# giech/usrp_nfc

Measured on AMD Instinct MI355X. Metric: IQ Msamples/s -> decoded bits (2 Msps stream), higher is better.
Workload: dtype f32 envelope / f64 window sums / u8 symbols; 1 GPU; configs[1]: Miller-only decode, synthetic IQ @2 Msps; input_kind=fc32 IQ, 8 B/sample (envelope computed in the kernel), samples_per_gpu=100000000, parallelism=time-chunk x1, edges_per_gpu=6627699, symbols_reader=3971547, symbols_tag=0, packets=101186, boundary_redos=0, exchange=none, stepping=sync, in_flight=1

## Files before the change

usrp_nfc_amd/csrc/host_context.h:

```cpp
#pragma once


namespace {

std::string g_create_error;

}

enum : int {
    TOT_RUNS = 0,
    TOT_EDGES = 8,
    TOT_DECMAP = 16,
    TOT_SPEC = 40,
    TOT_PKT0 = 72,
    TOT_PKT1 = 80,
    TOT_LAST2 = 88,
    TOT_NSYM = 96,
    TOT_CERT = 104,
    TOT_FRAME = 128,
    TOT_BYTES = 160
};

static_assert(sizeof(CertSummary) <= TOT_FRAME - TOT_CERT, "the verdict summary fits its slot of the totals");
struct DevState {
    Carry carry;
    EdgeCarry ecarry;
    DecCarry dcarry;
    uint8_t totals[TOT_BYTES];
    uint32_t seq[4];
};

constexpr size_t AHEAD_LDS_MAX = 96 * 1024;
constexpr int LEAN_STEPS_AHEAD = 4;
constexpr int NRING = 4;
constexpr int NSUB = 3;

namespace {
struct Switches {
    std::optional<std::string> debug_clk;
    std::optional<int> no_small, debug_bad_launch, debug_redo_submitted, debug, trace, trace_alloc, no_submit_ahead, wg, wg_rounds, wg_bulk, wg_rerun, wg_rowbal, wg_nr, wg_per_cu, wg_per_cu_ahead, wg_ex, lean, lean_rounds,
        lean_waves, edge_prefix, dec_spec, dec_runin, spin_wait, chunk_adapt, chunk_mult;
    std::optional<double> lean_gfac, lean_gmin, eps;
    std::optional<unsigned long> own_prefix_max;
    std::optional<std::pair<int, int>> wg_lone;
    std::optional<std::array<double, 3>> rowbal_f;
    std::optional<bool> ring_global;
};
inline Switches read_switches() {
    Switches s;
#ifdef NFC_TEST_HOOKS
    const struct { const char *name; std::optional<int> Switches::*at; } ints[] = {
        {"NFC_NO_SMALL", &Switches::no_small}, {"NFC_DEBUG_BAD_LAUNCH", &Switches::debug_bad_launch}, {"NFC_DEBUG_REDO_SUBMITTED", &Switches::debug_redo_submitted},
        {"NFC_DEBUG", &Switches::debug}, {"NFC_TRACE", &Switches::trace}, {"NFC_TRACE_ALLOC", &Switches::trace_alloc}, {"NFC_NO_SUBMIT_AHEAD", &Switches::no_submit_ahead},
        {"NFC_WG", &Switches::wg}, {"NFC_WG_ROUNDS", &Switches::wg_rounds}, {"NFC_WG_BULK", &Switches::wg_bulk},
        {"NFC_WG_RERUN", &Switches::wg_rerun}, {"NFC_WG_NR", &Switches::wg_nr}, {"NFC_WG_PER_CU", &Switches::wg_per_cu},
        {"NFC_WG_PER_CU_AHEAD", &Switches::wg_per_cu_ahead}, {"NFC_WG_EX", &Switches::wg_ex}, {"NFC_LEAN", &Switches::lean}, {"NFC_LEAN_ROUNDS", &Switches::lean_rounds},
        {"NFC_LEAN_WAVES", &Switches::lean_waves}, {"NFC_EDGE_PREFIX", &Switches::edge_prefix}, {"NFC_DEC_SPEC", &Switches::dec_spec}, {"NFC_DEC_RUNIN", &Switches::dec_runin},
        {"NFC_SPIN_WAIT", &Switches::spin_wait}, {"NFC_CHUNK_ADAPT", &Switches::chunk_adapt}, {"NFC_CHUNK_MULT", &Switches::chunk_mult}};
    const struct { const char *name; std::optional<double> Switches::*at; } reals[] = {
        {"NFC_LEAN_GFAC", &Switches::lean_gfac}, {"NFC_LEAN_GMIN", &Switches::lean_gmin}, {"NFC_EPS", &Switches::eps}};
    for (const auto &v : ints)
        if (const char *e = getenv(v.name)) s.*v.at = atoi(e);
    for (const auto &v : reals)
        if (const char *e = getenv(v.name)) s.*v.at = atof(e);
    if (const char *e = getenv("NFC_DEBUG_CLK")) s.debug_clk = e;
    if (const char *e = getenv("NFC_OWN_PREFIX_MAX")) s.own_prefix_max = strtoul(e, nullptr, 10);
    if (const char *e = getenv("NFC_WG_LONE")) {
        int a = 4, b = 64;
        if (sscanf(e, "%d,%d", &a, &b) >= 1) s.wg_lone = std::make_pair(a, b);
    }
    if (const char *e = getenv("NFC_WG_ROWBAL")) {
        std::array<double, 3> f{0.0, 1.0, 1.0};
        if (sscanf(e, "%lf,%lf,%lf", &f[0], &f[1], &f[2]) >= 2 && f[0] > 0.5 && f[0] < 1.5 && f[1] > 0.5 && f[1] < 1.5 && f[2] > 0.5 && f[2] < 1.5)
            s.rowbal_f = f;
        else s.wg_rowbal = atoi(e);
    }
    if (const char *e = getenv("NFC_RING")) {
        if (strcmp(e, "global") == 0) s.ring_global = true;
        else if (strcmp(e, "lds") == 0) s.ring_global = false;
    }
#endif
// ... 92 lines not shown
    uint32_t slot_next = 0;
    bool low_valid = false;
    size_t lean_lds_per_cu = 0;
    size_t ahead_lds_per_cu = 0;
    uint32_t stamp_b = 0;
    bool in_wait = false;
    uint32_t dbg_fast_waits = 0;
    uint32_t stats_redo_submitted = 0;
    Carry h_carry;
    EdgeCarry h_ecarry;
    DecCarry h_dcarry;
    uint64_t nseen = 0;

    DevBuf d_certinfo;
    DevBuf d_in, d_neg, d_pos, d_ringout[2], d_touched[2], d_info[2], d_ringin, d_meta, d_ver, d_cflags, d_list;
    DevBuf d_ecode, d_epos, d_eidx;
    bool edges_from_host = false;
    std::vector<nfc_edge> h_pushed;
    DevBuf d_states, d_sym[2], d_bits[2], d_pending[2][2], d_close_end[2],
        d_close_idx[2];
    DevBuf d_partials, d_partials2, d_aggs, d_faggs;
    DevBuf d_edge_rec;
    int edge_prefix = -1;
    DevBuf d_spec;
    DevBuf d_stage_bits[2], d_stage_cb[2], d_stage_ci[2], d_stage_q[2], d_stage_own;
    DevBuf d_pack;
    DevBuf d_gvtop;
    DevBuf d_seqout;
    uint32_t cap_edges = 0, cap_sym[2] = {0, 0};
    uint32_t alloc_edges = 0, alloc_sym[2] = {0, 0};
    uint64_t alloc_mark = 0;
    uint64_t cap_edges_floor = 0, cap_sym_floor[2] = {0, 0};
    double edge_rate = 0.125;
    double sym_rate[2] = {1.0, 2.0};
    int pend_cur = 0;
    std::vector<uint8_t> h_ver;
    std::vector<uint32_t> h_list;

    const void *last_in = nullptr;
    uint32_t last_n = 0, last_skip = 0;
    uint64_t last_g0 = 0;
    uint32_t n_edges = 0;
    uint32_t n_sym[2] = {0, 0}, n_close[2] = {0, 0}, n_bits[2] = {0, 0};
    bool have_outputs = false;
    nfc_stats stats;
    std::vector<nfc_packet> pk[2];
// ... 80 lines not shown
#define HIPCHK(c, call)                                                                              \
    do {                                                                                             \
        hipError_t e__ = (call);                                                                     \
        if (e__ != hipSuccess)                                                                       \
            return fail((c), NFC_ERR_DEVICE, "%s failed: %s (%s:%d)", #call, hipGetErrorString(e__), __FILE__, __LINE__); \
    } while (0)

int batch_ok(nfc_ctx *c, bool with_mirror) {
    LaunchError &le = launch_error();
    if (le.err != hipSuccess) {
        const LaunchError e = le;
        le = LaunchError{};
        return fail(c, NFC_ERR_DEVICE, "kernel launch failed: %s (%s:%d)", hipGetErrorString(e.err), e.file, e.line);
    }
    if (with_mirror && c->hs->seq[0] != c->batch_seq)
        return fail(c, NFC_ERR_DEVICE, "state mirror is stale (batch %u, mirror %u): a kernel of this batch did not run", c->batch_seq, c->hs->seq[0]);
    return NFC_OK;
}
#define BATCHCHK(c, with_mirror)                                   \
    do {                                                           \
        if (int rc__ = batch_ok((c), (with_mirror))) return rc__;  \
    } while (0)

void launch_fill_kind(nfc_ctx *c, const void *in, uint32_t n, int nchunks, int ring_idx = -1) {
    float *ring = c->d_ring[ring_idx < 0 ? c->ring_cur : ring_idx].as<float>();
    Carry *cr = dC(c);
    EdgeCarryInit eci{(int32_t *)dE(c), c->L % c->mx};
    uint8_t *ver = c->d_ver.as<uint8_t>();
    CertSummary *sum = (CertSummary *)(dT(c) + TOT_CERT);
    StateInit init;
    memset(&init, 0, sizeof init);
    int fresh = 0;
    if (c->state_dirty) {
        static_assert(offsetof(DevState, totals) <= sizeof init.words && offsetof(DevState, totals) % 4 == 0, "state head fits");
        DevState h;
        h.carry = c->dirty_carry;
        h.ecarry = c->dirty_ecarry;
        h.dcarry = c->dirty_dcarry;
        init.apply = 1;
        init.n_words = (int32_t)(offsetof(DevState, totals) / 4);
        memcpy(init.words, &h, offsetof(DevState, totals));
        init.dst = (uint32_t *)c->d_state.p;
        init.fill_ring = c->dirty_fill_ring ? 1 : 0;
        init.fill = c->dirty_fill;
        init.ring_len = c->Lpad;
        c->state_dirty = c->dirty_fill_ring = false;
        fresh = h.carry.stable == 0 && h.carry.filled == 0 && n >= (uint32_t)c->L && (void *)cr == c->d_state.p;
// ... 21 lines not shown
```

usrp_nfc_amd/csrc/host_threshold.h:

```cpp
#pragma once

namespace {

static bool sums_exact(const Carry &hc, int emin, int emax, uint32_t vtop) {
    int low = emin - 23;
    if (hc.ss_emin != 255) low = std::min(low, hc.ss_emin);
    float vtf;
    memcpy(&vtf, &vtop, 4);
    int high = 255 + 64;
    if (std::isfinite(vtf) && vtf >= 0.f) high = vtf > 0.f ? std::ilogb((double)vtf) + 127 : 0;
    high = std::max(high, hc.ss_emax);
    return (emax < 255) && (high - low <= 52);
}

static inline void eps_adapt(nfc_ctx *c, const CertSummary &s) {
    if (!c->dbg_trace) return;
    float w;
    memcpy(&w, &s.worst, 4);
    fprintf(stderr, "[nfc] eps %.5f: the speculation used %.5f of the window sum at most, %u chunks failed their certification\n", (double)c->eps, (double)w, s.n_fail);
}

static inline void cpu_relax() {
#if defined(__x86_64__) || defined(__i386__)
    __builtin_ia32_pause();
// ... 236 lines not shown
    P.h_gflags = h_gflags;
    P.h_gmin = h_gmin;
    P.h_gmax = h_gmax;
    return NFC_OK;
}

static void enqueue_pass0(nfc_ctx *c, const ThrPlan &P, ThrArgs &A, const Event *own_events = nullptr) {
    A.list = nullptr;
    A.nlist = 0;
    A.mode = 0;
    A.cert = P.d_cert;
    A.sum = (CertSummary *)(dT(c) + TOT_CERT);
    A.ksteps = P.form == ThrForm::Workgroup ? c->wg_rounds : c->lean_rounds;
    A.gfac = c->lean_gfac;
    A.gfloor = c->lean_gmin;
    A.blk = 1 << c->nfold;
    launch_threshold(c, P, ThrLaunch::Pass0, A, P.nch, own_events);
}
static void enqueue_certify(nfc_ctx *c, const ThrPlan &P, const ThrArgs &A, CertInfo *info, float *ring_out, CertSummary *sum) {
    NFC_LAUNCH(k_certify, dim3(cert_grid(A.nlist)), dim3(256), 0, c->st, A, P.d_cert, info, ring_out, dC(c), sum);
}

static int threshold_span(nfc_ctx *c, const void *d_in_all, uint32_t n_all, uint32_t skip_all, uint32_t base, const EdgeCarry &ec,
                          const std::function<int()> *ahead, bool *clean, bool *need_seq_out, bool *recut_out = nullptr) {
    bool ran_ahead = false;
    *clean = false;
    const int L = c->L;
    const uint32_t n = n_all - base;
    const uint32_t skip = skip_all > base ? skip_all - base : 0u;
    const void *d_in = (const char *)d_in_all + (size_t)base * c->in_bytes_per_sample;
    const uint64_t nseen = c->nseen + base;
    uint32_t passes = 0;
    ThrArgs A;
    ThrPlan P;
    if (int rc = thr_prepare(c, d_in, n, n_all, skip, base, nseen, ec, c->ring_cur, c->d_neg, c->d_pos, false, A, P)) return rc;
    const uint32_t nch = P.nch;
    const bool wg = P.form == ThrForm::Workgroup;
    uint8_t *d_cert = P.d_cert;
    const uint8_t *h_cert = P.h_cert, *h_gflags = P.h_gflags, *h_gmin = P.h_gmin, *h_gmax = P.h_gmax;

    launch_fill_kind(c, d_in, n, (int)nch);

    const bool force_seq = (c->P.flags & NFC_FLAG_FORCE_SEQUENTIAL) != 0 || L < STEP;
    bool need_seq = force_seq;
    if (!force_seq) {
        const bool lean = wg || P.form == ThrForm::Lean;
        const bool dbg_clk = lean && c->dbg_clk;
        if (dbg_clk) {
            HIPCHK(c, c->d_certinfo.ensure((size_t)nch * 32 * 5));
            A.dbg_clk = c->d_certinfo.as<unsigned long long>();
        }
        enqueue_pass0(c, P, A);
        if (dbg_clk) {
            std::vector<unsigned long long> h((size_t)nch * 4);
            HIPCHK(c, hipStreamSynchronize(c->st));
            HIPCHK(c, hipMemcpy(h.data(), c->d_certinfo.p, (size_t)nch * 32, hipMemcpyDeviceToHost));
            unsigned long long t0 = ~0ull, t1 = 0;
            double pro = 0, loop = 0, epi = 0, maxtot = 0, maxstart = 0;
            for (uint32_t k = 0; k < nch; k++) {
                t0 = std::min(t0, h[4 * k]);
                t1 = std::max(t1, h[4 * k + 3]);
            }
            for (uint32_t k = 0; k < nch; k++) {
                pro += (double)(h[4 * k + 1] - h[4 * k]);
                loop += (double)(h[4 * k + 2] - h[4 * k + 1]);
                epi += (double)(h[4 * k + 3] - h[4 * k + 2]);
                maxtot = std::max(maxtot, (double)(h[4 * k + 3] - h[4 * k]));
                maxstart = std::max(maxstart, (double)(h[4 * k] - t0));
            }
#ifdef NFC_WG_PROF
            if (wg) {
                std::vector<unsigned long long> pf((size_t)nch * 16);
                HIPCHK(c, hipMemcpy(pf.data(), (char *)c->d_certinfo.p + (size_t)nch * 32, (size_t)nch * 128, hipMemcpyDeviceToHost));
                double tk = 0, b1 = 0, b2 = 0, rr = 0;
                for (size_t k = 0; k < (size_t)nch * 4; k++) {
// ... 62 lines not shown
                    HIPCHK(c, mirror_async(c));
                } else {
                    stamped_last = c->timing < 2;
                }
                if (rc) return rc;
                ran_ahead = true;
            } else {
                launch_certify();
                flags_with_verdict = first_round && c->fine_left > 0;
                if (!first_round || flags_with_verdict) {
                    HIPCHK(c, hipMemcpyAsync(c->h_cflags.p, c->d_cflags.p, (size_t)4 * nch, hipMemcpyDeviceToHost, c->st));
                    HIPCHK(c, hipMemcpyAsync(P.h_gvtop, c->d_gvtop.p, (size_t)nch * 4, hipMemcpyDeviceToHost, c->st));
                }
                HIPCHK(c, mirror_async(c));
                if (first_round && ahead) {
                    const int rc = (*ahead)();
                    if (rc) return rc;
                    ran_ahead = true;
                }
            }
            if (stamped_last) HIPCHK(c, wait_for_stamp(c));
            else HIPCHK(c, hipStreamSynchronize(c->st));
            BATCHCHK(c, true);
            std::vector<uint32_t> failing;
            if (first_round) {
                memcpy(&summary, c->hs->totals + TOT_CERT, sizeof summary);
                if (base == 0) eps_adapt(c, summary);
                if (summary.n_fail == 0 && !dbg) {
                    have_summary = true;
                    break;
                }
                if (recut_out && c->fine_adapt && wg && c->fine_left == 0 && !c->P.chunk_samples && c->fine_mult > 1 &&
                    (uint64_t)summary.n_fail * 64u > (uint64_t)nch) {
                    *recut_out = true;
                    A.ver_zero = 0;
                    return NFC_OK;
                }
                if (!flags_with_verdict) HIPCHK(c, hipMemcpy(c->h_cflags.p, c->d_cflags.p, (size_t)4 * nch, hipMemcpyDeviceToHost));
            }
            if (first_round && lean && !h_cert[0]) failing.push_back(0);
            for (uint32_t k : c->h_list)
                if (!h_cert[k]) failing.push_back(k);
            if (c->dbg_trace) {
                fprintf(stderr, "[nfc] round %d: n_fail %u, %zu failing of %u pending (cert[0] %d):", rounds, summary.n_fail, failing.size(), np, (int)h_cert[0]);
                for (size_t i = 0; i < failing.size() && i < 12; i++) fprintf(stderr, " %u(%x)", failing[i], (unsigned)h_gflags[failing[i]]);
                int why[8] = {0};
// ... 173 lines not shown
    if (ec_out) {
        int32_t o[3];
        HIPCHK(c, hipStreamSynchronize(c->st));
        HIPCHK(c, hipMemcpy(o, c->d_seqout.p, sizeof o, hipMemcpyDeviceToHost));
        ec_out->state = o[0];
        ec_out->last_bit = o[1];
        ec_out->dur = o[2];
    }
    return NFC_OK;
}

int run_threshold(nfc_ctx *c, const void *d_in, uint32_t n, uint32_t skip, const std::function<int()> *ahead, bool *clean) {
    *clean = false;
    c->stats.threshold_passes = 0;
    c->stats.chunks_rerun = 0;
    c->stats.chunks_rerun_in_place = 0;
    c->stats.used_sequential = 0;
    const uint32_t span = (uint32_t)std::min<uint64_t>(((uint64_t)8 * c->L + STEP - 1) / STEP * STEP, 1u << 30);
    EdgeCarry ec = c->h_ecarry;
    uint32_t base = 0;
    for (int round = 0;; round++) {
        bool need_seq = false, span_clean = false;
        const bool optimistic = base == 0 && !(c->fine_adapt && c->fine_left > 0);
        bool recut = false;
        int rc = threshold_span(c, d_in, n, skip, base, ec, optimistic ? ahead : nullptr, &span_clean, &need_seq, &recut);
        if (rc) return rc;
        if (recut) {
            c->fine_left = 8;
            c->cert_pending = false;
            HIPCHK(c, hipMemsetAsync((char *)dC(c) + offsetof(Carry, fin_valid), 0, sizeof(int32_t), c->st));
            span_clean = false;
            rc = threshold_span(c, d_in, n, skip, base, ec, nullptr, &span_clean, &need_seq, nullptr);
            if (rc) return rc;
        }
        if (!need_seq) {
            *clean = span_clean && base == 0;
            if (c->fine_adapt) {
                if ((uint64_t)c->stats.chunks_rerun * 64u > (uint64_t)c->stats.n_chunks) c->fine_left = 8;
                else if (c->fine_left > 0) c->fine_left--;
            }
            return NFC_OK;
        }
        const bool forced = (c->P.flags & NFC_FLAG_FORCE_SEQUENTIAL) != 0 || c->L < STEP;
        const uint32_t left = n - base;
        if (forced || round >= 6 || left <= 4 * span) return sequential_span(c, d_in, skip, base, left, ec, nullptr);
        const int rs = sequential_span(c, d_in, skip, base, span, ec, &ec);
        if (rs) return rs;
        base += span;
    }
// ... 5 lines not shown
```

usrp_nfc_amd/csrc/nfc_amd.hip:

```cpp
#include <hip/hip_runtime.h>
#include <hip/hip_ext.h>

#include <algorithm>
#include <atomic>
#include <chrono>
#include <cmath>
#include <cstdarg>
#include <cstdio>
#include <cstdlib>
#include <cstring>
#include <string>
#include <thread>
#include <array>
#include <functional>
#include <memory>
#include <optional>
#include <vector>

#include "../../include/nfc_amd.h"
#include "launch_check.h"
#include "decode.hip.h"
#include "decoder_tables.h"
#include "edges.hip.h"
#include "scan.hip.h"
// ... 62 lines not shown
    c->use_small = sw.no_small ? 0 : 1;
    c->dbg_bad_launch = sw.debug_bad_launch.has_value();
    c->dbg_redo_submitted = sw.debug_redo_submitted.has_value();
    c->dbg_any = sw.debug.has_value();
    c->dbg_trace = sw.trace.has_value();
    devbuf_trace() = sw.trace_alloc.has_value();
    if (sw.debug_clk) {
        c->dbg_clk = true;
        c->dbg_clk_path = *sw.debug_clk;
    }
    c->dbg_no_submit_ahead = sw.no_submit_ahead.has_value();
    if (sw.wg) c->wg = *sw.wg != 0;
    if (sw.wg_rounds) c->wg_rounds = std::max(1, *sw.wg_rounds);
    if (sw.wg_bulk) c->wg_bulk = *sw.wg_bulk != 0;
    if (sw.wg_rerun) c->wg_rerun_lone = *sw.wg_rerun != 0;
    if (sw.wg_lone) c->wg_lone_max = std::max(0, sw.wg_lone->first), c->wg_lone_div = std::max(1, sw.wg_lone->second);
    if (sw.lean) c->lean = *sw.lean != 0;
    c->lean_rounds = 0;
    if (sw.lean_rounds) c->lean_rounds = std::max(1, *sw.lean_rounds);
    if (sw.lean_gfac) c->lean_gfac = (float)*sw.lean_gfac;
    if (sw.lean_gmin) c->lean_gmin = (float)*sw.lean_gmin;
    if (sw.own_prefix_max) c->own_prefix_max = (uint32_t)*sw.own_prefix_max;
    if (sw.edge_prefix) c->edge_prefix = *sw.edge_prefix != 0;
    if (sw.dec_spec) c->dec_spec = *sw.dec_spec != 0;
    if (sw.spin_wait) c->spin_wait = *sw.spin_wait != 0;
    if (sw.rowbal_f) memcpy(c->rowbal_f[0], sw.rowbal_f->data(), sizeof c->rowbal_f[0]), c->rowbal_set = true;
    if (sw.wg_rowbal) c->wg_rowbal = *sw.wg_rowbal != 0;
    if (sw.dec_runin) c->dec_runin = *sw.dec_runin >= 2048 ? 8 : (*sw.dec_runin >= 1024 ? 4 : 2);
    C = (C + STEP - 1) / STEP * STEP;
    c->C_min = C;
    c->lds_per_slot = (p->input_kind == NFC_IN_ENV_F32) ? 5 : 4;
    c->wpb = std::max(1, std::min(4, (int)(65536 / ((size_t)c->Lpad * c->lds_per_slot))));
    c->gring_ok = (size_t)c->Lpad * c->lds_per_slot > 12 * 1024 && c->L >= 2 * STEP;
    if (sw.ring_global) {
        if (*sw.ring_global && c->L >= 2 * STEP) c->gring_ok = c->gring_force = 1;
        else if (!*sw.ring_global) c->gring_ok = 0;
    }
    c->hi_plus = p->hi_val + 0.1;
    const double eps = std::ldexp(1.0, -48);
    auto band = [&](double v, double &a, double &b) {
        a = v - std::fabs(v) * eps;
        b = v + std::fabs(v) * eps;
    };
    band(p->lo_val, c->lo_a, c->lo_b);
    band(p->hi_val, c->hi_a, c->hi_b);
    auto sane = [](double v) { return v == 0 || (std::fabs(v) > 1e-100 && std::fabs(v) < 1e100); };
// ... 154 lines not shown
    }
    c->T.mil_map = c->d_mil_map.as<uint4>();
    c->T.man_map = c->d_man_map.as<uint2>();
    c->T.mil_step = c->d_mil_out.as<uint16_t>();
    c->T.man_step = c->d_man_out.as<uint16_t>();
    c->T.nd = c->mx + 1;
    c->T.reader = p->enable_reader ? 1 : 0;
    c->T.tag = p->enable_tag ? 1 : 0;
    for (int k = 0; k < 3; k++) c->dec_lds[k] = dec_table_bytes((DecLdsUser)k, c->T);
    CRT(c->d_state.ensure(sizeof(DevState)));
    CRT(c->hs_pin.ensure(sizeof(DevState)));
    c->hs = c->hs_pin.as<DevState>();
    memset(c->hs, 0, sizeof(DevState));
    CRT(hipHostGetDevicePointer(&c->hs_dev, c->hs, 0));
    for (int b = 0; b < NRING; b++) {
        CRT(c->d_ring[b].ensure((size_t)c->Lpad * 4));
        CRT(hipMemset(c->d_ring[b].p, 0, (size_t)c->Lpad * 4));
    }
    for (int b = 0; b < 2; b++) {
        CRT(c->d_pending[b][0].ensure(1024));
        CRT(c->d_pending[b][1].ensure(1024));
    }
    push_state(c, 1);
    CRT(hipStreamSynchronize(c->st));
    return NFC_OK;
}
#undef CRT
}

extern "C" {

int nfc_abi_version(void) { return NFC_AMD_ABI_VERSION; }

int nfc_plan_row_cut(uint32_t n, uint32_t C, uint32_t rs, uint32_t cus, uint32_t rows, const double *factors, uint32_t max_len, uint32_t out[10]) {
    if (!out || !rs || !C || !cus || (rows >= 2 && !factors)) return NFC_ERR_ARG;
    const RowCut t = (rows >= 2 && rows <= 4) ? plan_row_cut(n, C, rs, cus, rows, factors, max_len) : equal_cut(n, C, cus);
    for (int r = 0; r < 4; r++) {
        out[r] = t.row_len[r];
        out[4 + r] = t.row_start[r];
    }
    out[8] = t.row_div;
    out[9] = t.nch;
    return t.by_row ? 1 : 0;
}

int nfc_device_count(void) {
// ... 947 lines not shown
#ifdef NFC_GEN_PROF
extern "C" int nfc_debug_gen_prof(unsigned long long *out, int reset) {
    const size_t bytes = sizeof(unsigned long long) * 8192 * 8;
    if (hipMemcpyFromSymbol(out, HIP_SYMBOL(nfc::g_gen_prof), bytes) != hipSuccess) return -1;
    {
        unsigned long long ri[2] = {0, 0};
        if (hipMemcpyFromSymbol(ri, HIP_SYMBOL(nfc::g_row_iters), sizeof ri) == hipSuccess)
            fprintf(stderr, "[nfc] row_exact: %llu rows, %.2f iterations each\n", ri[0], ri[0] ? (double)ri[1] / (double)ri[0] : 0.0);
        void *q = nullptr;
        if (reset && hipGetSymbolAddress(&q, HIP_SYMBOL(nfc::g_row_iters)) == hipSuccess) (void)hipMemset(q, 0, sizeof ri);
    }
    if (reset) {
        void *p = nullptr;
        if (hipGetSymbolAddress(&p, HIP_SYMBOL(nfc::g_gen_prof)) != hipSuccess || hipMemset(p, 0, bytes) != hipSuccess) return -1;
    }
    return 0;
}
#endif
#ifdef NFC_TEST_HOOKS
extern "C" float nfc_debug_frames_ms(const nfc_ctx *c) { return c && c->frames_ready ? c->fr_ms : -1.f; }
extern "C" void nfc_debug_live_resources(uint64_t out[4]) {
    for (int k = 0; k < 4; k++) out[k] = nfc::live::count(k).load();
}
extern "C" int nfc_debug_dec_lds(const nfc_ctx *c, int which, uint32_t *dyn_bytes, int *wgs_per_cu) {
    if (!c || which < 0 || which > 2 || !dyn_bytes || !wgs_per_cu) return NFC_ERR_ARG;
    const bool lds = 4 * c->T.nd <= nfc::DEC_LDS_ROWS;
    const void *k = which == 0   ? (const void *)nfc::dec_spec_kernel(lds, c->T)
                    : which == 1 ? (lds ? (const void *)nfc::k_dec_reduce<true> : (const void *)nfc::k_dec_reduce<false>)
                                 : (lds ? (const void *)nfc::k_dec_apply<true> : (const void *)nfc::k_dec_apply<false>);
    *dyn_bytes = (uint32_t)c->dec_lds[which];
    if (hipSetDevice(c->P.device) != hipSuccess) return NFC_ERR_DEVICE;
    return hipOccupancyMaxActiveBlocksPerMultiprocessor(wgs_per_cu, k, nfc::SCAN_BLOCK, c->dec_lds[which]) == hipSuccess ? NFC_OK : NFC_ERR_DEVICE;
}
extern "C" int nfc_debug_dec_shapes(const nfc_ctx *c, uint32_t *out6) {
    if (!c || !out6) return NFC_ERR_ARG;
    out6[0] = (uint32_t)nfc::DEC_TILE;
    out6[1] = c->own_prefix_max;
    out6[2] = nfc::ST_CLOSES;
    out6[3] = (uint32_t)nfc::DEC_LDS_ROWS;
    out6[4] = (uint32_t)(nfc::DEC_RUNIN_MAX * nfc::SCAN_BLOCK);
    out6[5] = c->sym_own ? 1u : 0u;
    return NFC_OK;
}
#endif
```

usrp_nfc_amd/csrc/threshold.hip.h:

```cpp
#pragma once
#include <hip/hip_runtime.h>
#include <stdint.h>

#include <type_traits>

namespace nfc {

constexpr int STEP = 256;
constexpr int LL_NONE = -(1 << 30);
constexpr int MAX_FIX_ITERS = 80;
constexpr float RND_SUM = 2.44140625e-04f;

enum : int { IN_IQ_F32 = 0, IN_ENV_F32 = 1, IN_REAL_F32_SQ = 2, IN_I16_SQ = 3, IN_IQ_I16 = 4, IN_IQ_I8 = 5, IN_IQ_U8 = 6 };

#ifndef NFC_HDR_KERNEL_LINKAGE
#define NFC_HDR_KERNEL_LINKAGE
#endif

struct Carry {
    double ss;
    double delta;
    int32_t filled;
    int32_t stable;
    int32_t ss_emin;
// ... 10 lines not shown
        c.ss = c.ss_fin;
        c.fin_valid = 0;
    }
}

constexpr int KEY_NONE = INT32_MIN;

struct ChunkInfo {
    double ss_out;
    int32_t low_key;
    int32_t last_nonlow;
    uint32_t emin;
    uint32_t emax;
    uint32_t flags;
    uint32_t n_untouched;
};

struct RunMeta {
    float min_ss;
    float eps;
    int32_t nl_in, kl_in;
    uint32_t all_robust;
    uint32_t pad;
};

struct CertSummary;
struct ThrArgs {
    void *gring;
    const void *in;
    uint32_t n;
    uint32_t skip;
    uint32_t g0modL;
    int32_t L, Lpad, mx, C, nchunks;
    double lo, hi, hi_plus, lo_a, lo_b, hi_a, hi_b;
    int32_t bands_ok;
    int32_t fast_ok;
    float i16_scale;
    float eps;
    const float *ring_carry;
    const Carry *carry;
    int32_t nl0, kl0;
    const Carry *low_src;
    double lo_L, hi_L;
    int32_t fold_sh[6];
    int32_t probe_mid, probe_end;
    uint64_t selmask;
// ... 2 lines not shown
    ChunkInfo *info[2];
    const uint8_t *ver;
    float *ring_in;
    RunMeta *meta;
    uint8_t *gmin, *gmax, *gflags;
    uint32_t *gvtop;
    uint64_t *neg, *pos;
    const uint32_t *list;
    uint32_t nlist;
    int32_t mode;
    int32_t twords;
    int32_t off;
    int32_t nrows;
    uint8_t *cert;
    CertSummary *sum;
    int32_t ksteps;
    float gfac, gfloor;
    int32_t blk;
    int32_t ver_zero;
    int32_t wg_stage_rounds;
    unsigned long long *dbg_clk;
    uint32_t row_len[4], row_start[4], row_div;
    int C_max;
};
__device__ __forceinline__ void chunk_span(const ThrArgs &A, uint32_t c, uint32_t &m_chunk, uint32_t &len) {
    const uint32_t row = min(c / A.row_div, 3u);
    len = A.row_len[row];
    m_chunk = A.row_start[row] + (c - row * A.row_div) * len;
}

__device__ __forceinline__ int rfl(int v) { return __builtin_amdgcn_readfirstlane(v); }
__device__ __forceinline__ uint32_t rfl(uint32_t v) { return (uint32_t)__builtin_amdgcn_readfirstlane((int)v); }
__device__ __forceinline__ float rfl(float v) { return __int_as_float(__builtin_amdgcn_readfirstlane(__float_as_int(v))); }
__device__ __forceinline__ double rfl(double v) {
    return __hiloint2double(__builtin_amdgcn_readfirstlane(__double2hiint(v)), __builtin_amdgcn_readfirstlane(__double2loint(v)));
}
__device__ __forceinline__ bool uni(bool c) { return __builtin_amdgcn_readfirstlane((int)c) != 0; }
template <int CTRL, int ROWMASK>
__device__ __forceinline__ int dpp_i32(int ident, int v) {
    return __builtin_amdgcn_update_dpp(ident, v, CTRL, ROWMASK, 0xF, false);
}
__device__ __forceinline__ float wave_sum_f32(float v) {
    v += __int_as_float(dpp_i32<0x111, 0xF>(0, __float_as_int(v)));
    v += __int_as_float(dpp_i32<0x112, 0xF>(0, __float_as_int(v)));
    v += __int_as_float(dpp_i32<0x114, 0xF>(0, __float_as_int(v)));
    v += __int_as_float(dpp_i32<0x118, 0xF>(0, __float_as_int(v)));
    v += __int_as_float(dpp_i32<0x142, 0xA>(0, __float_as_int(v)));
// ... 1367 lines not shown
```

usrp_nfc_amd/csrc/threshold_wg.hip.h:

```cpp
#pragma once
#include "edges.hip.h"
#include "threshold_lean.hip.h"

namespace nfc {

constexpr int WG_WAVES = 4;
constexpr int wg_round_samples(int nr) { return 64 * nr * WG_WAVES; }
constexpr int WG_NR_MAX = 8;
#ifndef NFC_WG_FR
#define NFC_WG_FR 8
#endif
constexpr int wg_flush_rounds(int nr) { return nr == 4 ? NFC_WG_FR : NFC_WG_FR / 2; }
constexpr size_t wg_stage_bytes(int nr, int rounds) { return (size_t)rounds * (size_t)(2 * WG_WAVES * 2 * nr * 4); }
struct WgShared {
    uint32_t msk[3][WG_WAVES][4 * WG_NR_MAX + 4];
    uint32_t scr[2][WG_WAVES][8];
    int32_t fin[WG_WAVES][4];
    float4 acc[WG_WAVES][64];
    uint32_t flag[WG_WAVES];
    uint32_t cold[WG_WAVES][8];
    float bc[8];
};
constexpr size_t WG_SHARED_BYTES = (sizeof(WgShared) + 15) & ~(size_t)15;

// ... 114 lines not shown
    const unsigned long long bn = ~low_now & lane_lt;
    const int nl = bn ? rb + last_set(bn) : w_nl;
    int key = KEY_NONE;
    if (lw) {
        const int p = m - nl;
        const bool bad = (p > mx) && ((p - 1) % mx == 0);
        key = 2 * m + (bad ? 0 : 1);
    }
    const unsigned long long bl = low_now & lane_lt;
    const int kq = __shfl(key, bl ? last_set(bl) : 0, 64);
    const int kl = bl ? max(kq, w_kl) : w_kl;
    const bool st2 = (kl & 1) && (m - (kl >> 1)) <= mx + 1;
    int v = 0;
    if (lw) v = -1;
    else if (hg && !st2) v = 1;
    accm = __ballot(v == 0);
    lowm = low_now;
    posm = __ballot(v == 1);
    const unsigned long long nonlowf = ~low_now;
    w_nl = nonlowf ? rb + last_set(nonlowf) : w_nl;
    if (low_now) w_kl = max(w_kl, __builtin_amdgcn_readlane(key, last_set(low_now)));
}

template <int KIND, int NR, bool EX = false>
__global__ __launch_bounds__(256) void k_threshold_wg(ThrArgs A) {
    static_assert(!EX || NR == 4, "the samples of an exact round travel through sh->acc: sixteen rows");
    constexpr uint32_t STEPN = 64u * NR;
    constexpr int WG_ROUND = wg_round_samples(NR);
    extern __shared__ __attribute__((aligned(16))) unsigned char smem[];
    const int tid = (int)threadIdx.x;
    const int lane = tid & 63, wave = rfl(tid >> 6);
    const uint32_t c = A.list ? rfl(A.list[blockIdx.x]) : blockIdx.x;
    float *ring = (float *)smem;
    lean_lds_f *const rl = (lean_lds_f *)ring;
    WgShared *const sh = (WgShared *)(smem + (size_t)A.Lpad * 4);
    const int L = A.L;
    const int mx = A.mx;
    uint32_t m_chunk_v, chunk_len_v;
    chunk_span(A, c, m_chunk_v, chunk_len_v);
    const uint32_t m_chunk = rfl(m_chunk_v), chunk_len = rfl(chunk_len_v);
    const uint32_t n1 = min(A.n, m_chunk + chunk_len);
    const uint32_t m_start = max(m_chunk, A.skip);
    constexpr int RB = LeanRaw<KIND>::BYTES;
    const uint32_t wbase0 = m_chunk + STEPN * (uint32_t)wave;
    const char *const in_first = (const char *)A.in + (size_t)wbase0 * RB;
    const uint32_t voff = (uint32_t)lane * (uint32_t)RB;
    bool primed = false;
    if (m_chunk >= m_start && m_chunk + (uint32_t)wg_round_samples(NR) <= n1) {
        wg_load_step<KIND, NR>(voff, in_first);
        primed = true;
    }
    const Carry cr = *A.carry;
    uint64_t *const neg_p = A.neg, *const pos_p = A.pos;
    const uintptr_t plane_of_lane = (lane >= 2 * NR) ? (uintptr_t)pos_p : (uintptr_t)neg_p;
    const int plane_dword = (lane >= 2 * NR) ? lane - 2 * NR : lane;
    const float i16s = A.i16_scale;
    const unsigned long long lane_lt = (1ull << lane) - 1ull;
    int scr_par = 0;
    auto wg_gather = [&](const uint32_t (&v)[8], int k, uint32_t (&out)[WG_WAVES][8]) __attribute__((always_inline)) {
        if (lane == 0)
            for (int i = 0; i < k; i++) sh->scr[scr_par][wave][i] = v[i];
        wg_barrier();
        for (int w = 0; w < WG_WAVES; w++)
            for (int i = 0; i < k; i++) out[w][i] = rfl(sh->scr[scr_par][w][i]);
        scr_par ^= 1;
    };

    for (int i = tid; i < (int)(sizeof(sh->msk) / 4); i += 256) ((uint32_t *)sh->msk)[i] = 0u;
    if (lane == 0) {
        sh->cold[wave][0] = (uint32_t)LL_NONE;
        sh->cold[wave][1] = (uint32_t)LL_NONE;
        sh->cold[wave][2] = 0xFFFFFFFFu;
        sh->cold[wave][3] = 0u;
        sh->cold[wave][4] = sh->cold[wave][5] = 0x7F61B1E6u;
    }
// ... 5 lines not shown
#pragma unroll
            for (int f = 0; f < 6; f++) t &= t >> A.fold_sh[f];
            hit |= t & A.selmask;
        }
        return hit != 0ull;
    };
    unsigned long long clk0 = 0, clk1 = 0, clk2 = 0;
#ifdef NFC_WG_PROF
    unsigned long long pf_take = 0, pf_b1 = 0, pf_b2 = 0, pf_rounds = 0, pf_t = 0;
#define WG_PF_BEGIN() pf_t = clock64()
#define WG_PF_END(acc) acc += clock64() - pf_t
#else
#define WG_PF_BEGIN() ((void)0)
#define WG_PF_END(acc) ((void)0)
#endif
    if (A.dbg_clk) clk0 = clock64();

    uint32_t emin = 255u, emax = 0u, vtop0 = 0u;
    int nl_in, kl_in;
    float ssf, eps = 0.f;
    {
        double ss0;
        if (c == 0) {
            for (int s = tid; s < L; s += 256) ring[s] = A.ring_carry[s];
            ss0 = cr.ss;
            nl_in = carried_nl(A);
            kl_in = carried_kl(A);
            wg_barrier();
        } else if (A.mode == 1) {
            double part = 0;
            for (int s = tid; s < L; s += 256) {
                const float v = resolve_slot(A, (int)c, s);
                ring[s] = v;
                part += (double)v;
            }
            const double ps = wave_sum_f64(part);
            uint32_t v[8], g[WG_WAVES][8];
            v[0] = (uint32_t)__double2loint(ps);
            v[1] = (uint32_t)__double2hiint(ps);
            wg_gather(v, 2, g);
            double tot = 0;
            for (int w = 0; w < WG_WAVES; w++) tot += __hiloint2double((int)g[w][1], (int)g[w][0]);
            ss0 = tot + cr.delta;
            resolve_low_state(A, (int)c, nl_in, kl_in);
        } else {
            eps = A.eps;
            const uint32_t w0 = m_chunk - (uint32_t)L;
            const uint32_t slot0 = (A.g0modL + w0) % (uint32_t)L;
// ... 73 lines not shown
            ss0 = tot + cr.delta;
        }
        ssf = rfl((float)ss0);
        float *rin = A.ring_in + (size_t)c * L;
        for (int s = tid; s < L; s += 256) {
            const float v = ring[s];
            __builtin_nontemporal_store(v, rin + s);
            vtop0 = max(vtop0, __float_as_uint(v));
            ring[s] = __uint_as_float(__float_as_uint(v) | 0x80000000u);
            if (v != 0.f) {
                const uint32_t e = max(f32_expfield(v), 1u);
                emin = min(emin, e);
                emax = max(emax, e);
            }
        }
        uint32_t v[8], g[WG_WAVES][8];
        v[0] = wave_max_u32(vtop0);
        v[1] = wave_min_u32(emin);
        v[2] = wave_max_u32(emax);
        wg_gather(v, 3, g);
        vtop0 = max(max(g[0][0], g[1][0]), max(g[2][0], g[3][0]));
        emin = min(min(g[0][1], g[1][1]), min(g[2][1], g[3][1]));
        emax = max(max(g[0][2], g[1][2]), max(g[2][2], g[3][2]));
    }
    nl_in = rfl(nl_in);
    kl_in = rfl(kl_in);

    if (A.dbg_clk) clk1 = clock64();
    bool good_run = A.fast_ok != 0;
    if constexpr (KIND == IN_ENV_F32) good_run = good_run && vtop0 < 0x7F800000u;
    uint32_t why = good_run ? 0u : 1u;
    float min_ss = 3.0e38f;
    uint32_t vmin = 0xFFFFFFFFu, vmax = vtop0;
    const float etaD = 1.0f - 9.5367431640625e-07f;
    const float slU = 1.0f + 3.814697265625e-06f;
    const float loLf = (float)A.lo_L, hiLf = (float)A.hi_L;
    uint32_t slot_step = (A.g0modL + wbase0) % (uint32_t)L;
    const uint32_t slot_adv = (uint32_t)WG_ROUND % (uint32_t)L;
    float b_acc = 0.f, dl_acc = 0.f;
    float tlo = 0.f, thi = 0.f;
    float dlo = 3.0e38f, dhi = 3.0e38f;
    uint32_t xlo_acc = 0x7F7FFFFFu, xhi_acc = 0u;
    int lz_base = LL_NONE;
    int rounds_since_sync = 0;
    float xkeep[NR], snap[NR];
    uint32_t snap_slot = 0u, st_off_round = 0u, c_snap[4] = {0u, 0u, 0u, 0u};
// ... 834 lines not shown
            if (found) {
                const int koff = ll - (s1 + 1);
                if (koff > 0 && (koff % mx) == 0) chunk_kl = 2 * ll;
            } else {
                good_run = false;
                why = 3u;
            }
        }
    }

#ifdef NFC_EX_PRINTF
    if (EX && tid == 0) printf("chunk %u: %d of %d rounds exact (codes %x, first %d last %d, %d trips) good %d why %u; cycles: prologue %llu rounds %llu (in place %llu) summary-so-far %llu\n", c, ex_count, n_rounds, ex_codes, ex_first, ex_last, ex_trips, (int)good_run, why, ex_t1 - ex_t0, ex_ta - ex_t1, ex_tx, clock64() - ex_ta);
#endif
    if (A.dbg_clk) clk2 = clock64();
    const uint32_t all_robust = good_run ? 1u : 0u;
    if (c == 0 && tid == 0 && A.mode == 0) {
        A.cert[0] = good_run ? 1 : 0;
        if (!good_run) atomicAdd(&A.sum->n_fail, 1u);
    }
    {
        uint32_t v[8], g[WG_WAVES][8];
        v[0] = min(wave_min_u32(vmin), rfl(sh->cold[wave][2]));
        v[1] = max(wave_max_u32(vmax), rfl(sh->cold[wave][3]));
        const int vb_new = (A.mode == 1) ? 1 - (int)A.ver[c] : (int)A.ver[c];
        float *ro = (vb_new ? A.ring_out[1] : A.ring_out[0]) + (size_t)c * L;
        uint32_t *to = (vb_new ? A.touched[1] : A.touched[0]) + (size_t)c * A.twords;
        uint32_t untouched = 0;
        for (int sbase = 64 * wave; sbase < A.twords * 32; sbase += 256) {
            const int s = sbase + lane;
            const float rv = (s < L) ? ring[s] : 0.f;
            const bool t = (s < L) && !(__float_as_uint(rv) >> 31);
            const unsigned long long bal = __ballot(t);
            if (s < L) {
                __builtin_nontemporal_store(fabsf(rv), ro + s);
                if (!t) untouched++;
            }
            const int w = sbase >> 5;
            if (lane == 0) {
                to[w] = (uint32_t)bal;
                if (w + 1 < A.twords) to[w + 1] = (uint32_t)(bal >> 32);
            }
        }
        v[2] = (uint32_t)wave_sum_f32((float)untouched);
        wg_gather(v, 3, g);
        vmin = min(min(g[0][0], g[1][0]), min(g[2][0], g[3][0]));
        vmax = max(max(g[0][1], g[1][1]), max(g[2][1], g[3][1]));
        untouched = g[0][2] + g[1][2] + g[2][2] + g[3][2];
// ... 49 lines not shown
```

Before: 447,900 Msamples/s.

## Fold fresh-stream fill launch into the threshold workgroup kernel

On a fresh stream batch, the separate fill kernel launch is skipped. Chunk 0 of the threshold kernel now computes the initial envelope ring, its sum, the state words and the version bytes itself, and the host passes the dirty state through the kernel arguments. If the kernel finds that the sum would not be exact, the host redoes the span through the old path. This removes one kernel launch and its state upload per fresh batch, at the cost of a larger argument block and a possible second pass.

Result: no change. 452,400 Msamples/s (median of 6 runs) (+1.0%).

```diff
diff --git a/usrp_nfc_amd/csrc/host_context.h b/usrp_nfc_amd/csrc/host_context.h
--- a/usrp_nfc_amd/csrc/host_context.h
+++ b/usrp_nfc_amd/csrc/host_context.h
@@ -39,7 +39,7 @@
 struct Switches {
     std::optional<std::string> debug_clk;
     std::optional<int> no_small, debug_bad_launch, debug_redo_submitted, debug, trace, trace_alloc, no_submit_ahead, wg, wg_rounds, wg_bulk, wg_rerun, wg_rowbal, wg_nr, wg_per_cu, wg_per_cu_ahead, wg_ex, lean, lean_rounds,
-        lean_waves, edge_prefix, dec_spec, dec_runin, spin_wait, chunk_adapt, chunk_mult;
+        lean_waves, edge_prefix, dec_spec, dec_runin, spin_wait, chunk_adapt, chunk_mult, prep_launch;
     std::optional<double> lean_gfac, lean_gmin, eps;
     std::optional<unsigned long> own_prefix_max;
     std::optional<std::pair<int, int>> wg_lone;
@@ -56,7 +56,8 @@
         {"NFC_WG_RERUN", &Switches::wg_rerun}, {"NFC_WG_NR", &Switches::wg_nr}, {"NFC_WG_PER_CU", &Switches::wg_per_cu},
         {"NFC_WG_PER_CU_AHEAD", &Switches::wg_per_cu_ahead}, {"NFC_WG_EX", &Switches::wg_ex}, {"NFC_LEAN", &Switches::lean}, {"NFC_LEAN_ROUNDS", &Switches::lean_rounds},
         {"NFC_LEAN_WAVES", &Switches::lean_waves}, {"NFC_EDGE_PREFIX", &Switches::edge_prefix}, {"NFC_DEC_SPEC", &Switches::dec_spec}, {"NFC_DEC_RUNIN", &Switches::dec_runin},
-        {"NFC_SPIN_WAIT", &Switches::spin_wait}, {"NFC_CHUNK_ADAPT", &Switches::chunk_adapt}, {"NFC_CHUNK_MULT", &Switches::chunk_mult}};
+        {"NFC_SPIN_WAIT", &Switches::spin_wait}, {"NFC_CHUNK_ADAPT", &Switches::chunk_adapt}, {"NFC_CHUNK_MULT", &Switches::chunk_mult},
+        {"NFC_PREP_LAUNCH", &Switches::prep_launch}};
     const struct { const char *name; std::optional<double> Switches::*at; } reals[] = {
         {"NFC_LEAN_GFAC", &Switches::lean_gfac}, {"NFC_LEAN_GMIN", &Switches::lean_gmin}, {"NFC_EPS", &Switches::eps}};
     for (const auto &v : ints)
@@ -195,6 +196,8 @@
     DevBuf d_partials, d_partials2, d_aggs, d_faggs;
     DevBuf d_edge_rec;
     int edge_prefix = -1;
+    bool prep_launch = false;
+    uint64_t fill_launches = 0;
     DevBuf d_spec;
     DevBuf d_stage_bits[2], d_stage_cb[2], d_stage_ci[2], d_stage_q[2], d_stage_own;
     DevBuf d_pack;
@@ -321,7 +324,32 @@
         if (int rc__ = batch_ok((c), (with_mirror))) return rc__;  \
     } while (0)
 
+inline bool fresh_stream_batch(const nfc_ctx *c, uint32_t n) {
+    return c->state_dirty && c->dirty_carry.stable == 0 && c->dirty_carry.filled == 0 && n >= (uint32_t)c->L;
+}
+void prep_fresh_args(nfc_ctx *c, ThrArgs &A) {
+    static_assert(offsetof(DevState, totals) <= sizeof A.pf.words && offsetof(DevState, totals) % 4 == 0, "state head fits");
+    static_assert(offsetof(DevState, carry) == 0, "the carry heads the state block");
+    DevState h;
+    h.carry = c->dirty_carry;
+    h.ecarry = c->dirty_ecarry;
+    h.dcarry = c->dirty_dcarry;
+    A.prep = 1;
+    A.pf.ring = c->d_ring[c->ring_cur].as<float>();
+    A.pf.state = (uint32_t *)c->d_state.p;
+    A.pf.ver = c->d_ver.as<uint8_t>();
+    A.pf.n_words = (int32_t)(offsetof(DevState, totals) / 4);
+    A.pf.ring_pad = c->dirty_fill_ring ? 1 : 0;
+    A.pf.ecarry_word = (int32_t)(offsetof(DevState, ecarry) / 4);
+    A.pf.dur0 = c->L % c->mx;
+    A.pf.sum_word = (int32_t)((offsetof(DevState, totals) + TOT_CERT) / 4);
+    A.pf.seq_word = (int32_t)(offsetof(DevState, seq) / 4);
+    A.pf.seq = c->batch_seq;
+    memcpy(A.pf.words, &h, offsetof(DevState, totals));
+}
+
 void launch_fill_kind(nfc_ctx *c, const void *in, uint32_t n, int nchunks, int ring_idx = -1) {
+    c->fill_launches++;
     float *ring = c->d_ring[ring_idx < 0 ? c->ring_cur : ring_idx].as<float>();
     Carry *cr = dC(c);
     EdgeCarryInit eci{(int32_t *)dE(c), c->L % c->mx};
diff --git a/usrp_nfc_amd/csrc/host_threshold.h b/usrp_nfc_amd/csrc/host_threshold.h
--- a/usrp_nfc_amd/csrc/host_threshold.h
+++ b/usrp_nfc_amd/csrc/host_threshold.h
@@ -282,7 +282,7 @@
 }
 
 static int threshold_span(nfc_ctx *c, const void *d_in_all, uint32_t n_all, uint32_t skip_all, uint32_t base, const EdgeCarry &ec,
-                          const std::function<int()> *ahead, bool *clean, bool *need_seq_out, bool *recut_out = nullptr) {
+                          const std::function<int()> *ahead, bool *clean, bool *need_seq_out, bool *recut_out = nullptr, bool *reprep_out = nullptr) {
     bool ran_ahead = false;
     *clean = false;
     const int L = c->L;
@@ -299,9 +299,16 @@
     uint8_t *d_cert = P.d_cert;
     const uint8_t *h_cert = P.h_cert, *h_gflags = P.h_gflags, *h_gmin = P.h_gmin, *h_gmax = P.h_gmax;
 
-    launch_fill_kind(c, d_in, n, (int)nch);
-
     const bool force_seq = (c->P.flags & NFC_FLAG_FORCE_SEQUENTIAL) != 0 || L < STEP;
+    const bool prep_fresh = reprep_out && !c->prep_launch && wg && !force_seq && base == 0 && fresh_stream_batch(c, n);
+    const bool fresh_fill_ring = c->dirty_fill_ring;
+    if (prep_fresh) {
+        prep_fresh_args(c, A);
+        c->state_dirty = c->dirty_fill_ring = false;
+    } else {
+        launch_fill_kind(c, d_in, n, (int)nch);
+    }
+
     bool need_seq = force_seq;
     if (!force_seq) {
         const bool lean = wg || P.form == ThrForm::Lean;
@@ -311,6 +318,7 @@
             A.dbg_clk = c->d_certinfo.as<unsigned long long>();
         }
         enqueue_pass0(c, P, A);
+        A.prep = 0;
         if (dbg_clk) {
             std::vector<unsigned long long> h((size_t)nch * 4);
             HIPCHK(c, hipStreamSynchronize(c->st));
@@ -419,6 +427,13 @@
             if (stamped_last) HIPCHK(c, wait_for_stamp(c));
             else HIPCHK(c, hipStreamSynchronize(c->st));
             BATCHCHK(c, true);
+            if (first_round && prep_fresh && c->hs->seq[2] == c->batch_seq) {
+                c->state_dirty = true;
+                c->dirty_fill_ring = fresh_fill_ring;
+                *reprep_out = true;
+                A.ver_zero = 0;
+                return NFC_OK;
+            }
             std::vector<uint32_t> failing;
             if (first_round) {
                 memcpy(&summary, c->hs->totals + TOT_CERT, sizeof summary);
@@ -638,9 +653,15 @@
     for (int round = 0;; round++) {
         bool need_seq = false, span_clean = false;
         const bool optimistic = base == 0 && !(c->fine_adapt && c->fine_left > 0);
-        bool recut = false;
-        int rc = threshold_span(c, d_in, n, skip, base, ec, optimistic ? ahead : nullptr, &span_clean, &need_seq, &recut);
+        bool recut = false, reprep = false;
+        int rc = threshold_span(c, d_in, n, skip, base, ec, optimistic ? ahead : nullptr, &span_clean, &need_seq, &recut, &reprep);
         if (rc) return rc;
+        if (reprep) {
+            c->cert_pending = false;
+            span_clean = false;
+            rc = threshold_span(c, d_in, n, skip, base, ec, nullptr, &span_clean, &need_seq, &recut, nullptr);
+            if (rc) return rc;
+        }
         if (recut) {
             c->fine_left = 8;
             c->cert_pending = false;
diff --git a/usrp_nfc_amd/csrc/nfc_amd.hip b/usrp_nfc_amd/csrc/nfc_amd.hip
--- a/usrp_nfc_amd/csrc/nfc_amd.hip
+++ b/usrp_nfc_amd/csrc/nfc_amd.hip
@@ -108,6 +108,7 @@
     if (sw.lean_gmin) c->lean_gmin = (float)*sw.lean_gmin;
     if (sw.own_prefix_max) c->own_prefix_max = (uint32_t)*sw.own_prefix_max;
     if (sw.edge_prefix) c->edge_prefix = *sw.edge_prefix != 0;
+    if (sw.prep_launch) c->prep_launch = *sw.prep_launch != 0;
     if (sw.dec_spec) c->dec_spec = *sw.dec_spec != 0;
     if (sw.spin_wait) c->spin_wait = *sw.spin_wait != 0;
     if (sw.rowbal_f) memcpy(c->rowbal_f[0], sw.rowbal_f->data(), sizeof c->rowbal_f[0]), c->rowbal_set = true;
@@ -308,6 +309,7 @@
         CRT(c->d_pending[b][1].ensure(1024));
     }
     push_state(c, 1);
+    push_state(c);
     CRT(hipStreamSynchronize(c->st));
     return NFC_OK;
 }
@@ -1301,6 +1303,7 @@
 extern "C" void nfc_debug_live_resources(uint64_t out[4]) {
     for (int k = 0; k < 4; k++) out[k] = nfc::live::count(k).load();
 }
+extern "C" uint64_t nfc_debug_fill_launches(const nfc_ctx *c) { return c ? c->fill_launches : 0; }
 extern "C" int nfc_debug_dec_lds(const nfc_ctx *c, int which, uint32_t *dyn_bytes, int *wgs_per_cu) {
     if (!c || which < 0 || which > 2 || !dyn_bytes || !wgs_per_cu) return NFC_ERR_ARG;
     const bool lds = 4 * c->T.nd <= nfc::DEC_LDS_ROWS;
diff --git a/usrp_nfc_amd/csrc/threshold.hip.h b/usrp_nfc_amd/csrc/threshold.hip.h
--- a/usrp_nfc_amd/csrc/threshold.hip.h
+++ b/usrp_nfc_amd/csrc/threshold.hip.h
@@ -56,6 +56,20 @@
     int32_t nl_in, kl_in;
     uint32_t all_robust;
     uint32_t pad;
+};
+
+struct PrepFresh {
+    float *ring;
+    uint32_t *state;
+    uint8_t *ver;
+    int32_t n_words;
+    int32_t ring_pad;
+    int32_t ecarry_word;
+    int32_t dur0;
+    int32_t sum_word;
+    int32_t seq_word;
+    uint32_t seq;
+    uint32_t words[32];
 };
 
 struct CertSummary;
@@ -104,7 +118,10 @@
     unsigned long long *dbg_clk;
     uint32_t row_len[4], row_start[4], row_div;
     int C_max;
+    int32_t prep;
+    PrepFresh pf;
 };
+static_assert(sizeof(ThrArgs) <= 1024, "the threshold kernels' argument block stays far below the 4 KB kernel-argument limit");
 __device__ __forceinline__ void chunk_span(const ThrArgs &A, uint32_t c, uint32_t &m_chunk, uint32_t &len) {
     const uint32_t row = min(c / A.row_div, 3u);
     len = A.row_len[row];
diff --git a/usrp_nfc_amd/csrc/threshold_wg.hip.h b/usrp_nfc_amd/csrc/threshold_wg.hip.h
--- a/usrp_nfc_amd/csrc/threshold_wg.hip.h
+++ b/usrp_nfc_amd/csrc/threshold_wg.hip.h
@@ -160,6 +160,62 @@
     if (low_now) w_kl = max(w_kl, __builtin_amdgcn_readlane(key, last_set(low_now)));
 }
 
+template <int KIND>
+__device__ __noinline__ double wg_fill_fresh(const void *in, float i16_scale, int L, int Lpad, float *gring, int ring_pad) {
+    extern __shared__ __attribute__((aligned(16))) unsigned char smem[];
+    float *const ring = (float *)smem;
+    WgShared *const sh = (WgShared *)(smem + (size_t)Lpad * 4);
+    const int tid = (int)threadIdx.x, lane = tid & 63, wave = tid >> 6;
+    double part = 0;
+    for (int i0 = 0; i0 < L; i0 += 2048) {
+        typename RawOf<KIND>::T rw[8];
+#pragma unroll
+        for (int k = 0; k < 8; k++) {
+            const int i = i0 + 256 * k + tid;
+            rw[k] = (i < L) ? load_raw<KIND>(in, (size_t)i) : raw_zero<KIND>();
+        }
+#pragma unroll
+        for (int k = 0; k < 8; k++) {
+            const int i = i0 + 256 * k + tid;
+            if (i < L) {
+                const float x = env_of<KIND>(rw[k], i16_scale);
+                ring[i] = x;
+                gring[i] = x;
+                part += (double)x;
+            }
+        }
+    }
+    if (ring_pad)
+        for (int i = L + tid; i < Lpad; i += 256) gring[i] = 0.f;
+    const double ps = wave_sum_f64(part);
+    if (lane == 0) {
+        sh->scr[1][wave][0] = (uint32_t)__double2loint(ps);
+        sh->scr[1][wave][1] = (uint32_t)__double2hiint(ps);
+    }
+    wg_barrier();
+    double tot = 0;
+    for (int w = 0; w < WG_WAVES; w++) tot += __hiloint2double((int)sh->scr[1][w][1], (int)sh->scr[1][w][0]);
+    return rfl(tot);
+}
+__device__ __noinline__ void wg_store_fresh(Carry nc, double S, uint32_t emin, uint32_t emax, int L, uint32_t *state, int ecarry_word,
+                                            int dur0, int sum_word, int seq_word, uint32_t seq) {
+    int lg = 0;
+    while ((1 << lg) < L) lg++;
+    const bool exact = (emax < 255u) && ((int)emax + 2 + lg - ((int)emin - 23) <= 52);
+    state[seq_word] = seq;
+    state[seq_word + 2] = exact ? 0u : seq;
+    *(CertSummary *)(state + sum_word) = CertSummary{0u, 255u, 0u, 0u, 0u, 0u};
+    if (!exact) return;
+    nc.filled = L;
+    nc.ss = S;
+    nc.stable = 1;
+    batch_guard(nc, S, emin, emax);
+    *(Carry *)state = nc;
+    state[ecarry_word] = 0u;
+    state[ecarry_word + 1] = 0u;
+    state[ecarry_word + 2] = (uint32_t)dur0;
+}
+
 template <int KIND, int NR, bool EX = false>
 __global__ __launch_bounds__(256) void k_threshold_wg(ThrArgs A) {
     static_assert(!EX || NR == 4, "the samples of an exact round travel through sh->acc: sixteen rows");
@@ -188,7 +244,12 @@
         wg_load_step<KIND, NR>(voff, in_first);
         primed = true;
     }
-    const Carry cr = *A.carry;
+    const bool prep = !EX && A.prep != 0;
+    struct { double ss, delta; } cr = {0.0, 0.0};
+    if (!prep) {
+        cr.ss = A.carry->ss;
+        cr.delta = A.carry->delta;
+    }
     uint64_t *const neg_p = A.neg, *const pos_p = A.pos;
     const uintptr_t plane_of_lane = (lane >= 2 * NR) ? (uintptr_t)pos_p : (uintptr_t)neg_p;
     const int plane_dword = (lane >= 2 * NR) ? lane - 2 * NR : lane;
@@ -240,8 +301,12 @@
     {
         double ss0;
         if (c == 0) {
-            for (int s = tid; s < L; s += 256) ring[s] = A.ring_carry[s];
-            ss0 = cr.ss;
+            if (prep) {
+                ss0 = wg_fill_fresh<KIND>(A.in, A.i16_scale, L, A.Lpad, A.pf.ring, A.pf.ring_pad);
+            } else {
+                for (int s = tid; s < L; s += 256) ring[s] = A.ring_carry[s];
+                ss0 = cr.ss;
+            }
             nl_in = carried_nl(A);
             kl_in = carried_kl(A);
             wg_barrier();
@@ -361,6 +426,24 @@
         vtop0 = max(max(g[0][0], g[1][0]), max(g[2][0], g[3][0]));
         emin = min(min(g[0][1], g[1][1]), min(g[2][1], g[3][1]));
         emax = max(max(g[0][2], g[1][2]), max(g[2][2], g[3][2]));
+        if constexpr (!EX) {
+            if (prep) {
+                if (tid == 0) A.pf.ver[c] = 0;
+                if (c == 0) {
+                    constexpr int CW = (int)(sizeof(Carry) / 4);
+                    static_assert(sizeof(Carry) % 4 == 0 && sizeof(Carry) <= sizeof(A.pf.words), "the carry heads the state block");
+                    if (tid >= CW && tid < A.pf.n_words && (tid < A.pf.ecarry_word || tid >= A.pf.ecarry_word + 3)) A.pf.state[tid] = A.pf.words[tid];
+                    if (tid == 0) {
+                        Carry nc;
+                        uint32_t cw[CW];
+#pragma unroll
+                        for (int k = 0; k < CW; k++) cw[k] = A.pf.words[k];
+                        memcpy(&nc, cw, sizeof nc);
+                        wg_store_fresh(nc, ss0, emin, emax, L, A.pf.state, A.pf.ecarry_word, A.pf.dur0, A.pf.sum_word, A.pf.seq_word, A.pf.seq);
+                    }
+                }
+            }
+        }
     }
     nl_in = rfl(nl_in);
     kl_in = rfl(kl_in);
@@ -1241,7 +1324,7 @@
         uint32_t v[8], g[WG_WAVES][8];
         v[0] = min(wave_min_u32(vmin), rfl(sh->cold[wave][2]));
         v[1] = max(wave_max_u32(vmax), rfl(sh->cold[wave][3]));
-        const int vb_new = (A.mode == 1) ? 1 - (int)A.ver[c] : (int)A.ver[c];
+        const int vb_new = (A.mode == 1) ? 1 - (int)A.ver[c] : ((!EX && A.prep != 0) ? 0 : (int)A.ver[c]);
         float *ro = (vb_new ? A.ring_out[1] : A.ring_out[0]) + (size_t)c * L;
         uint32_t *to = (vb_new ? A.touched[1] : A.touched[0]) + (size_t)c * A.twords;
         uint32_t untouched = 0;
```
